# njspix/frender

Hardware: AMD Instinct MI355X
Metric: M reads/sec scanned+classified (96 samples, 8+8bp, n=1) at 1/2/4/8 MI355X (higher is better)
Workload: dtype u8; 1 GPU; BASELINE config 2: 100000000 SYN-v1 reads/GPU, 96 samples, 8+8bp, n=1, R=8 (74 B/record), decoded FASTQ resident in HBM; reads_per_gpu=100000000, bytes_per_record=74, samples=96, nsubs=1, rc=False, unique_codes=1383958, table_checksum=a89b0e2c6adb2921, parallelism=1 GPU

## Files before the change

frender_amd/_lib.py:

```python
from __future__ import annotations

import ctypes as C
import os

import numpy as np

from . import _runtime

torch = None
if _runtime.USE_TORCH:
    try:
        import torch
    except Exception:
        torch = None

HERE = os.path.dirname(os.path.abspath(__file__))
LIB_PATH = os.environ.get("FRENDER_HIP_LIB", os.path.join(HERE, "libfrender_hip.so"))


def source_tree_hash() -> str:
    import hashlib

    h = hashlib.sha256()
    csrc = os.path.join(HERE, "csrc")
# ... 14 lines not shown


class FrenderError(RuntimeError):
    pass


class FileStats(C.Structure):
    _fields_ = [("records", C.c_uint64), ("lines", C.c_uint64), ("new_keys", C.c_uint64),
                ("exotic", C.c_uint64), ("error", C.c_int32), ("utf8_bad", C.c_int32),
                ("error_offset", C.c_uint64)]


class Timing(C.Structure):
    _fields_ = [("scan_launches", C.c_uint64), ("scan_bytes", C.c_uint64), ("scan_ms", C.c_double),
                ("last_scan_ms", C.c_double), ("classify_ms", C.c_double), ("finalize_ms", C.c_double),
                ("log_ms", C.c_double)]


class Tuning(C.Structure):
    _fields_ = [("size", C.c_uint32), ("grid", C.c_int32), ("flush_at", C.c_uint32), ("cold_cap", C.c_uint32),
                ("log", C.c_int32), ("log_min", C.c_uint32), ("log_hot", C.c_uint32), ("chunk_tiles", C.c_uint32),
                ("chunk_tiles_heavy", C.c_uint32), ("ramp", C.c_int32), ("ramp_up_s", C.c_uint32),
                ("ramp_down_s", C.c_uint32), ("ramp_down_pct", C.c_uint32), ("ramp_down_pct_h", C.c_uint32),
                ("spec_commit", C.c_int32), ("nbr", C.c_int32), ("ovf_cap", C.c_uint64)]


if not os.path.exists(LIB_PATH):
    raise ImportError(f"frender_amd: HIP library {LIB_PATH} is not built (run __graft_entry__.build())")
lib = C.CDLL(LIB_PATH)

P = C.c_void_p
u64p = C.POINTER(C.c_uint64)
_SIGS = {
    "fr_create": (P, [C.c_int, C.c_uint64, C.c_uint64]),
    "fr_tuning_defaults": (None, [C.POINTER(Tuning)]),
    "fr_create_tuned": (P, [C.c_int, C.c_uint64, C.c_uint64, C.POINTER(Tuning)]),
    "fr_destroy": (None, [P]),
    "fr_last_error": (C.c_char_p, [P]),
    "fr_get_timing": (C.c_int, [P, C.POINTER(Timing)]),
    "fr_sync": (C.c_int, [P]),
    "fr_set_timing": (C.c_int, [P, C.c_int]),
    "fr_get_diag": (C.c_int, [P, P, C.c_int]),
    "fr_set_sheet": (C.c_int, [P, C.c_int, P, P, P, P, P, P, C.c_int, P, P, P, C.c_int]),
    "fr_reset": (C.c_int, [P]),
    "fr_begin_file": (C.c_int, [P, C.c_int64]),
    "fr_begin_file_at": (C.c_int, [P, C.c_int64, C.c_uint64, C.c_int64]),
    "fr_feed": (C.c_int, [P, P, C.c_uint64]),
# ... 837 lines not shown
```

frender_amd/csrc/fr_api.hip:

```cpp
#include <hip/hip_runtime.h>

#include <algorithm>
#include <cstddef>
#include <cstdio>
#include <cstdlib>
#include <cstring>
#include <string>
#include <thread>
#include <unordered_map>
#include <vector>

#include "../../include/frender_amd.h"
#include "fr_internal.h"

using namespace fr;

static void pinned_copy(u8* dst, const u8* src, u64 n) {
    constexpr u64 PART = 16ull << 20;
    const unsigned hw = std::max(1u, std::thread::hardware_concurrency());
    const u64 k = std::min<u64>({8, hw, n / PART});
    if (k < 2) {
        std::memcpy(dst, src, n);
        return;
    }
    std::vector<std::thread> t;
    const u64 per = (n + k - 1) / k;
    for (u64 i = 1; i < k; ++i) {
        const u64 b = i * per, e = std::min(n, b + per);
        if (b < e) t.emplace_back([=] { std::memcpy(dst + b, src + b, e - b); });
    }
    std::memcpy(dst, src, std::min(n, per));
    for (auto& x : t) x.join();
}

struct fr_ctx {
    int device = 0;
    GSlot* snap = nullptr;
    u64 snap_cap = 0;
    hipStream_t stream = nullptr;
    hipStream_t copy = nullptr;
    std::string err;
    int grid = 0;
    u32 flush_at = NS * 3 / 4;
    u64* cold = nullptr;
    u32 cold_cap = 8192;
    LogEntry* log = nullptr;
    u64 log_cap = 0;
    u32 log_rcap = 0;
    LogEntry* log_sub = nullptr;
    u32 log_scap = 0;
    void* log_temp = nullptr;
    size_t log_temp_bytes = 0;
    u32 log_min = 0;
    u32 log_hot = 0xFFFFFFFFu;
    uint4* rare = nullptr;

    DevState* st = nullptr;
    DevState* h_st = nullptr;
    DevState* h_zero = nullptr;
    u8* h_byte = nullptr;
    u64* h_fin = nullptr;
    HostMirror* h_mir = nullptr;
    HostMirror* d_mir = nullptr;
// ... 168 lines not shown
    while (p < x) p <<= 1;
    return p;
}

static hipError_t fill_async(fr_ctx* ctx, void* dst, int value, size_t bytes) {
    ctx->n_fills++;
    return hipMemsetAsync(dst, value, bytes, ctx->stream);
}

static hipError_t copy_async(fr_ctx* ctx, void* dst, const void* src, size_t bytes, hipMemcpyKind kind) {
    ctx->n_copies++;
    return hipMemcpyAsync(dst, src, bytes, kind, ctx->stream);
}

static int read_state(fr_ctx* ctx) {
    if (ctx->st_fresh && !ctx->st_pending) return FR_OK;
    CK(copy_async(ctx, ctx->h_st, ctx->st, sizeof(DevState), hipMemcpyDeviceToHost));
    CK(hipStreamSynchronize(ctx->stream));
    ctx->st_pending = false;
    ctx->st_fresh = true;
    return FR_OK;
}

static int grow_table(fr_ctx* ctx, bool force_bigger) {
    int rc = read_state(ctx);
    if (rc) return rc;
    const u64 nkeys = ctx->h_st->n_keys;
    const u64 novf = std::min<u64>(ctx->h_st->n_overflow, ctx->tab.ovf_cap);
    if (force_bigger || (nkeys + novf) * 2 > ctx->nslots) {
        u64 ns = ctx->nslots;
        while ((nkeys + novf) * 4 > ns) ns <<= 1;
        if (ns == ctx->nslots) ns <<= 1;
        GSlot* ns_slots = nullptr;
        CK(dalloc(&ns_slots, ns));
        CK(launch_table_init(ns_slots, ns, nullptr, ctx->stream));
        Table t = ctx->tab;
        t.slots = ns_slots;
        t.mask = ns - 1;
        CK(launch_rehash(t, ctx->st, ctx->tab.slots, ctx->nslots, ctx->stream));
        CK(hipStreamSynchronize(ctx->stream));
        CK(hipFree(ctx->tab.slots));
        ctx->tab = t;
        ctx->nslots = ns;
    }
    if (novf) {
        Overflow* old = ctx->tab.ovf;
        Overflow* fresh = nullptr;
        CK(dalloc(&fresh, ctx->tab.ovf_cap));
        ctx->tab.ovf = fresh;
        CK(fill_async(ctx, &ctx->st->n_overflow, 0, sizeof(u64)));
        CK(launch_reinsert_overflow(ctx->tab, ctx->st, old, novf, ctx->stream));
        ctx->st_fresh = false;
        CK(hipStreamSynchronize(ctx->stream));
        CK(hipFree(old));
    }
// ... 318 lines not shown
extern "C" {

void fr_tuning_defaults(fr_tuning* t) {
    if (!t) return;
    const fr_ctx d{};
    std::memset(t, 0, sizeof(*t));
    t->size = sizeof(fr_tuning);
    t->grid = 0;
    t->flush_at = d.flush_at;
    t->cold_cap = d.cold_cap;
    t->log = 1;
    t->log_min = d.log_min;
    t->log_hot = d.log_hot;
    t->chunk_tiles = d.chunk_tiles;
    t->chunk_tiles_heavy = d.chunk_tiles_heavy;
    t->ramp = d.ramp ? 1 : 0;
    t->ramp_up_s = d.ramp_up_s;
    t->ramp_down_s = d.ramp_down_s;
    t->ramp_down_pct = d.ramp_down_pct;
    t->ramp_down_pct_h = d.ramp_down_pct_h;
    t->spec_commit = d.spec_ok ? 1 : 0;
    t->nbr = d.nbr_enabled ? 1 : 0;
    t->ovf_cap = 0;
}

fr_ctx* fr_create(int device, uint64_t chunk_bytes, uint64_t table_slots) {
    return fr_create_tuned(device, chunk_bytes, table_slots, nullptr);
}

fr_ctx* fr_create_tuned(int device, uint64_t chunk_bytes, uint64_t table_slots, const fr_tuning* tuning) {
    fr_tuning t;
    fr_tuning_defaults(&t);
    if (tuning) {
        const size_t n = std::min<size_t>(std::max<uint32_t>(tuning->size, sizeof(uint32_t)), sizeof(fr_tuning));
        std::memcpy((char*)&t + sizeof(uint32_t), (const char*)tuning + sizeof(uint32_t), n - sizeof(uint32_t));
    }
    fr_ctx* ctx = new fr_ctx();
    ctx->device = device;
    auto bad = [&](const char* what, hipError_t e) {
        ctx->err = std::string(what) + ": " + hipGetErrorString(e);
        return ctx;
    };
    hipError_t e;
    if ((e = hipSetDevice(device)) != hipSuccess) return bad("hipSetDevice", e);
    if ((e = hipStreamCreateWithFlags(&ctx->stream, hipStreamNonBlocking)) != hipSuccess) return bad("stream", e);
    if ((e = hipStreamCreateWithFlags(&ctx->copy, hipStreamNonBlocking)) != hipSuccess) return bad("stream", e);
    hipDeviceProp_t prop;
    if ((e = hipGetDeviceProperties(&prop, device)) != hipSuccess) return bad("props", e);
    const int per_cu = chunk_occupancy();
    ctx->grid = t.grid > 0 ? t.grid : prop.multiProcessorCount * per_cu;
    ctx->flush_at = std::min<u32>(t.flush_at, NS);
    ctx->nbr_enabled = t.nbr != 0;
    ctx->cold_cap = std::max<u32>(1024, t.cold_cap);
    ctx->log_min = t.log_min;
    ctx->log_hot = std::max<u32>(1, t.log_hot);
    ctx->chunk_tiles = std::max<u32>(2, t.chunk_tiles);
    ctx->chunk_tiles_heavy = std::max<u32>(2, t.chunk_tiles_heavy);
    ctx->ramp = t.ramp != 0;
    ctx->ramp_up_s = std::max<u32>(1, t.ramp_up_s);
    ctx->ramp_down_s = std::max<u32>(1, t.ramp_down_s);
    ctx->ramp_down_pct = std::min<u32>(100, std::max<u32>(1, t.ramp_down_pct));
    ctx->ramp_down_pct_h = std::min<u32>(100, std::max<u32>(1, t.ramp_down_pct_h));
    ctx->spec_ok = t.spec_commit != 0;
    if ((e = dalloc(&ctx->cold, 2ull * ctx->cold_cap * (u64)ctx->grid)) != hipSuccess) return bad("cold lists", e);
    if ((e = dalloc(&ctx->rare, (u64)RARE_RING * (u64)ctx->grid)) != hipSuccess) return bad("rare rings", e);

    ctx->chunk_bytes = chunk_bytes ? ((chunk_bytes + TILE - 1) / TILE) * TILE : (256ull << 20);
    if (ctx->chunk_bytes > RANGE_MAX) ctx->chunk_bytes = RANGE_MAX;
    ctx->ring_bytes = std::min<u64>(ctx->chunk_bytes, HOST_CHUNK_MAX);
// ... 35 lines not shown
    if ((e = dalloc(&ctx->tab.slots, ctx->nslots)) != hipSuccess) return bad("table", e);
    ctx->tab.mask = ctx->nslots - 1;
    ctx->tab.ovf_cap = t.ovf_cap ? std::max<u64>(t.ovf_cap, 1024) : (1ull << 22);
    ctx->tab.pres_cap = 1ull << 22;
    ctx->tab.exo_cap = 1ull << 20;
    ctx->tab.exo_pool_cap = 64ull << 20;
    if ((e = dalloc(&ctx->tab.ovf, ctx->tab.ovf_cap)) != hipSuccess) return bad("overflow", e);
    if ((e = dalloc(&ctx->tab.pres, ctx->tab.pres_cap)) != hipSuccess) return bad("presence", e);
    if ((e = dalloc(&ctx->tab.exo_ord, ctx->tab.exo_cap)) != hipSuccess) return bad("exotic", e);
    if ((e = dalloc(&ctx->tab.exo_off, ctx->tab.exo_cap)) != hipSuccess) return bad("exotic", e);
    if ((e = dalloc(&ctx->tab.exo_len, ctx->tab.exo_cap)) != hipSuccess) return bad("exotic", e);
    if ((e = dalloc(&ctx->tab.exo_pool, ctx->tab.exo_pool_cap)) != hipSuccess) return bad("exotic", e);
    for (int i = 0; i < 2; ++i) {
        if ((e = hipHostMalloc((void**)&ctx->pin[i], ctx->ring_bytes, hipHostMallocDefault)) != hipSuccess)
            return bad("pinned ring", e);
        if ((e = dalloc(&ctx->dbuf[i], ctx->ring_bytes + 64)) != hipSuccess) return bad("device ring", e);
        if ((e = hipEventCreateWithFlags(&ctx->copied[i], hipEventDisableTiming)) != hipSuccess) return bad("event", e);
        if ((e = hipEventCreateWithFlags(&ctx->consumed[i], hipEventDisableTiming)) != hipSuccess)
            return bad("event", e);
        if ((e = hipEventRecord(ctx->consumed[i], ctx->stream)) != hipSuccess) return bad("event", e);
    }
    if ((e = dalloc(&ctx->d_counter, 1)) != hipSuccess) return bad("counter", e);
    if (fr_reset(ctx) != FR_OK) return ctx;
    ctx->err.clear();
    return ctx;
}

void fr_destroy(fr_ctx* ctx) {
    if (!ctx) return;
    if (ctx->infl) fr_infl_destroy(ctx->infl);
    (void)hipSetDevice(ctx->device);
    if (ctx->stream) (void)hipStreamSynchronize(ctx->stream);
    if (ctx->copy) (void)hipStreamSynchronize(ctx->copy);
    void* dev[] = {ctx->st, ctx->d_tab, ctx->tiles, ctx->tab.slots, ctx->tab.ovf, ctx->tab.pres, ctx->tab.exo_ord,
                   ctx->tab.exo_off, ctx->tab.exo_len, ctx->tab.exo_pool, ctx->dbuf[0], ctx->dbuf[1], ctx->d_sheet,
                   ctx->d_keys, ctx->d_counts, ctx->d_first, ctx->d_keys_s, ctx->d_counts_s,
                   ctx->d_first_s, ctx->d_pos, ctx->d_perm, ctx->d_rank, ctx->d_counter, ctx->d_temp, ctx->d_bins, ctx->d_binbase, ctx->d_arr, ctx->d_rows, ctx->d_pres_u,
                   ctx->d_pres_f, ctx->d_pres_c, ctx->d_m1, ctx->d_m2, ctx->d_row, ctx->d_rm2, ctx->d_rrow, ctx->d_cls, ctx->d_rcls,
                   ctx->d_errw, ctx->d_errf, ctx->d_nbr, ctx->cold, ctx->rare, ctx->chunk_info, ctx->log, ctx->log_sub, ctx->log_temp,
                   ctx->snap};
    for (void* p : dev)
        if (p) (void)hipFree(p);
    if (ctx->h_st) (void)hipHostFree(ctx->h_st);
    if (ctx->h_zero) (void)hipHostFree(ctx->h_zero);
    if (ctx->h_byte) (void)hipHostFree(ctx->h_byte);
    if (ctx->h_fin) (void)hipHostFree(ctx->h_fin);
    if (ctx->h_mir) (void)hipHostFree(ctx->h_mir);
    if (ctx->fin_e0) (void)hipEventDestroy(ctx->fin_e0);
    if (ctx->fin_e1) (void)hipEventDestroy(ctx->fin_e1);
    if (ctx->cls_e0) (void)hipEventDestroy(ctx->cls_e0);
    if (ctx->cls_e1) (void)hipEventDestroy(ctx->cls_e1);
    if (ctx->h_sheet) (void)hipHostFree(ctx->h_sheet);
    if (ctx->h_tab) (void)hipHostFree(ctx->h_tab);
    for (int i = 0; i < 2; ++i) {
        if (ctx->pin[i]) (void)hipHostFree(ctx->pin[i]);
        if (ctx->copied[i]) (void)hipEventDestroy(ctx->copied[i]);
        if (ctx->consumed[i]) (void)hipEventDestroy(ctx->consumed[i]);
    }
    for (auto e : ctx->ev_a) (void)hipEventDestroy(e);
    for (auto e : ctx->ev_b) (void)hipEventDestroy(e);
    for (auto e : ctx->ev_l) (void)hipEventDestroy(e);
    if (ctx->st_ev) (void)hipEventDestroy(ctx->st_ev);
    if (ctx->stream) (void)hipStreamDestroy(ctx->stream);
    if (ctx->copy) (void)hipStreamDestroy(ctx->copy);
    delete ctx;
}

const char* fr_last_error(const fr_ctx* ctx) { return ctx ? ctx->err.c_str() : "null context"; }

int fr_get_diag(fr_ctx* ctx, uint64_t* out, int n) {
    if (int src = settle_finalize(ctx)) return src;
    int rc = read_state(ctx);
    if (rc) return rc;
    const DevState& s = *ctx->h_st;
    const uint64_t v[] = {s.spin_max,   s.spin_total, s.n_keys,   s.n_overflow, s.n_presence, s.n_exotic,
                          (uint64_t)ctx->grid, ctx->nslots, s.stamp[0], s.stamp[1], s.stamp[2], s.stamp[3],
                          s.stamp[4],  s.stamp[5],  s.stamp[6], s.stamp[7], ctx->spec_replays, ctx->exo_replays,
                          s.heavy[ctx->par] ? ctx->chunk_tiles_heavy : ctx->chunk_tiles,
                          s.heavy_launches, ctx->big_rollbacks, ctx->feed_fold_max, ctx->feed_fold_over, ctx->feed_step,
                          ctx->n_fills, ctx->n_copies};
    for (int i = 0; i < n && i < (int)(sizeof(v) / sizeof(v[0])); ++i) out[i] = v[i];
    return FR_OK;
}

int fr_sync(fr_ctx* ctx) {
    CK(hipStreamSynchronize(ctx->stream));
    CK(hipStreamSynchronize(ctx->copy));
    return settle_finalize(ctx);
}

int fr_get_timing(fr_ctx* ctx, fr_timing* out) {
    CK(hipStreamSynchronize(ctx->stream));
    if (int src = settle_finalize(ctx)) return src;
    double tot = 0, last = 0, lg = 0;
    for (size_t i = 0; i < ctx->ev_used; ++i) {
        float ms = 0, ml = 0;
        CK(hipEventElapsedTime(&ms, ctx->ev_a[i], ctx->ev_b[i]));
        CK(hipEventElapsedTime(&ml, ctx->ev_b[i], ctx->ev_l[i]));
        tot += ms;
        last = ms;
        lg += ml;
    }
    out->log_ms = lg;
    out->scan_launches = ctx->scan_launches;
    out->scan_bytes = ctx->scan_bytes;
    out->scan_ms = tot;
    out->last_scan_ms = last;
    out->classify_ms = ctx->classify_ms;
    out->finalize_ms = ctx->finalize_ms;
    return FR_OK;
// ... 67 lines not shown
    ctx->d_name = (int32_t*)(d + o_name);
    ctx->d_cp1 = with_cp ? (u32*)(d + o_cp1) : nullptr;
    ctx->d_cp2 = with_cp ? (u32*)(d + o_cp2) : nullptr;
    ctx->d_cp2rc = with_cp ? (u32*)(d + o_cp2rc) : nullptr;
    ctx->d_cpl1 = with_cp ? (int32_t*)(d + o_l1) : nullptr;
    ctx->d_cpl2 = with_cp ? (int32_t*)(d + o_l2) : nullptr;
    ctx->d_canon = (int32_t*)(d + o_canon);
    ctx->cp_stride = with_cp ? cp_stride : 0;
    ctx->S = S;
    ctx->n_names = n_names;
    auto common = [&](const int32_t* l) {
        if (S == 0) return -1;
        for (int i = 1; i < S; ++i)
            if (l[i] != l[0]) return -2;
        return (int)l[0];
    };
    ctx->L1u = common(idx1_len);
    ctx->L2u = common(idx2_len);
    return FR_OK;
}

int fr_reset(fr_ctx* ctx) {
    if (int src = settle_finalize(ctx)) return src;
    CK(hipSetDevice(ctx->device));
    CK(hipStreamSynchronize(ctx->copy));
    ctx->n_fills = ctx->n_copies = 0;
    if (ctx->st_pending) CK(hipStreamSynchronize(ctx->stream));
    CK(launch_table_init(ctx->tab.slots, ctx->nslots, ctx->st, ctx->stream));
    *ctx->h_st = *ctx->h_zero;
    ctx->st_fresh = true;
    ctx->perfile_clean = true;
    ctx->fold_zero = true;
    ctx->scanning = true;
    ctx->file_open = false;
    ctx->file_tag = 0;
    ctx->first_tag = 0;
    ctx->pres_defer_tag = 0;
    ctx->merged = false;
    ctx->max_file_bytes = 0;
    ctx->par = 0;
    ctx->U = 0;
    ctx->n_pres = 0;
    ctx->n_exo = 0;
    ctx->exo_index.clear();
    ctx->exo_str.clear();
    ctx->exo_codes.clear();
    ctx->exo_pres_code.clear();
    ctx->exo_pres_file.clear();
    ctx->exo_pres_count.clear();
    ctx->last_valid = false;
    ctx->ev_used = 0;
// ... 31 lines not shown
    ctx->file_tag = (u32)file_index + 1u;
    if (!ctx->first_tag) ctx->first_tag = ctx->file_tag;
    ctx->file_offset = byte_base;
    ctx->file_base = byte_base;
    ctx->max_records = max_records > 0 ? max_records : 0;
    ctx->last_byte = -1;
    ctx->carry.clear();
    ctx->sample_done = false;
    ctx->par = 0;
    ctx->file_open = true;
    return FR_OK;
}

static int check_sample(fr_ctx* ctx) {
    if (ctx->max_records <= 0) return FR_OK;
    int rc = read_state(ctx);
    if (rc) return rc;
    const u64 lines = ctx->h_st->lines[ctx->par];
    if (lines + 3 >= 4ull * (u64)ctx->max_records) ctx->sample_done = true;
    return FR_OK;
}

static int ship_slot(fr_ctx* ctx, int slot, u64 n) {
    CK(hipStreamWaitEvent(ctx->copy, ctx->consumed[slot], 0));
    CK(hipMemcpyAsync(ctx->dbuf[slot], ctx->pin[slot], n, hipMemcpyHostToDevice, ctx->copy));
    CK(hipEventRecord(ctx->copied[slot], ctx->copy));
    CK(hipStreamWaitEvent(ctx->stream, ctx->copied[slot], 0));
    int rc = launch_range(ctx, ctx->dbuf[slot], n, n, 1, 0, 0);
    if (rc) return rc;
    CK(hipEventRecord(ctx->consumed[slot], ctx->stream));
    ctx->used[slot] = true;
    return FR_OK;
}

int fr_feed(fr_ctx* ctx, const uint8_t* data, uint64_t len) {
    if (!ctx->file_open) return fail(ctx, FR_ERR_INVALID, "fr_feed: no open file");
    ctx->host_feed = true;
    if (ctx->sample_done) return FR_SAMPLE_DONE;
    if (len) ctx->last_byte = data[len - 1];
    u64 done = 0;
    while (done < len) {
        const int slot = ctx->cur;
        if (ctx->used[slot]) CK(hipEventSynchronize(ctx->copied[slot]));
        u8* pin = ctx->pin[slot];
        const u64 nc = ctx->carry.size();
        if (nc >= ctx->ring_bytes) return fail(ctx, FR_ERR_CAPACITY, "a line is longer than the chunk size");
// ... 50 lines not shown
    const double big_range = (double)std::min<u64>(ctx->chunk_bytes, len);
    const bool fold_room = (u64)ctx->feed_fold_over * 64 <= ctx->feed_fold_max && ctx->feed_step > 0 &&
                           (double)ctx->feed_fold_max * big_range <= 0.85 * AGG_LNS * (double)ctx->feed_step;
    bool big = spec && (!ctx->feed_logged || fold_room) && ctx->feed_keys != ~0ull &&
               (saved.n_keys + ctx->feed_keys) * 2 <= ctx->nslots;
    bool spec_now = spec;
    u64 step = 0, lim_room = ~0ull;
    int last_b = -1;
    for (int attempt = 0; attempt < 12; ++attempt) {
        const bool zero_fold = !ctx->fold_zero;
        bool mirrored = false;
        const u64 lim = std::min<u64>(big ? ctx->chunk_bytes : std::min<u64>(ctx->chunk_bytes, RANGE_FIRST_MAX),
                                      lim_room);
        const u64 nr = (len + lim - 1) / lim;
        step = nr ? (len + nr - 1) / nr : 0;
        ctx->spec_commit = spec_now ? 1u : 0u;
        for (u64 off = 0; off < len; off += step) {
            const u64 n = std::min<u64>(step, len - off);
            rc = launch_range(ctx, dev_data + off, n, len - off, off == 0 ? 1 : 0, 1, off ? 1 : 0, 0,
                              off + n == len, &mirrored, zero_fold && off == 0);
            if (rc) break;
        }
        ctx->spec_commit = 0;
        if (!rc && mirrored) {
            rc = take_mirror(ctx);
            last_b = (int)(ctx->h_mir->last_byte & 0xFFu);
        } else if (!rc) {
            if (len) CK(copy_async(ctx, ctx->h_byte, dev_data + len - 1, 1, hipMemcpyDeviceToHost));
            rc = read_state(ctx);
            if (!rc && len) last_b = *ctx->h_byte;
        }
        if (rc) break;
        const bool spec_bad = spec_now && ctx->h_st->spec_fail;
        const bool room_bad = spec && (ctx->h_st->cap_flags & 2u) && step > RANGE_ROOM_MIN;
        if (!spec_bad && !room_bad) break;
        if (room_bad) {
            big = false;
            lim_room = std::max<u64>(RANGE_ROOM_MIN, ((step / 8) + TILE - 1) / TILE * TILE);
            ctx->grow_sync = true;
            ctx->big_rollbacks++;
        } else {
            spec_now = false;
        }
        if (ctx->nslots != snap_slots) {
            GSlot* fresh = nullptr;
            if ((rc = (dalloc(&fresh, snap_slots) == hipSuccess) ? FR_OK : fail(ctx, FR_ERR_DEVICE, "rollback alloc")))
// ... 79 lines not shown
    if (rc) return fail(ctx, rc, std::string("fr_feed_bgzf: ") + fr_infl_last_error(ctx->infl));
    if (!ok) return FR_OK;
    rc = fr_feed_device(ctx, dev, len);
    if (rc) return rc;
    *decoded = 1;
    if (members) *members = n;
    if (bytes) *bytes = len;
    return FR_OK;
}

int fr_end_file(fr_ctx* ctx, fr_file_stats* out) {
    if (!ctx->file_open) return fail(ctx, FR_ERR_INVALID, "fr_end_file: no open file");
    if (!ctx->carry.empty() && !ctx->sample_done) {
        const int slot = ctx->cur;
        if (ctx->used[slot]) CK(hipEventSynchronize(ctx->copied[slot]));
        std::memcpy(ctx->pin[slot], ctx->carry.data(), ctx->carry.size());
        const u64 n = ctx->carry.size();
        ctx->carry.clear();
        int rc = ship_slot(ctx, slot, n);
        if (rc) return rc;
        ctx->cur ^= 1;
    }
    ctx->carry.clear();
    CK(hipStreamSynchronize(ctx->copy));
    int rc = ctx->host_feed ? settle_exotic(ctx) : FR_OK;
    if (rc) return rc;
    ctx->last_valid = false;
    rc = grow_table(ctx, false);
    if (rc) return rc;
    const bool defer = ctx->file_tag == ctx->first_tag && !ctx->merged && ctx->pres_before == 0 &&
                       ctx->h_st->n_presence == 0;
    if (!defer) {
        rc = ensure_presence_cap(ctx);
        if (rc) return rc;
        ctx->st_fresh = false;
        CK(launch_presence_scan(ctx->tab.slots, ctx->nslots, ctx->file_tag, ctx->tab.pres, ctx->tab.pres_cap,
                                ctx->st, ctx->stream));
    }
    rc = read_state(ctx);
    if (rc) return rc;
    const DevState& s = *ctx->h_st;
    if (s.spin_fail) return fail(ctx, FR_ERR_DEVICE, "tally look-back exceeded its spin bound");
    if (s.cap_flags) return fail(ctx, FR_ERR_CAPACITY, "a device list overflowed (flags " + std::to_string(s.cap_flags) + ")");
    u64 lines = s.lines[ctx->par];
    const bool ended = ctx->last_byte == '\n' || ctx->last_byte == '\r';
    if (ctx->last_byte >= 0 && !ended && !ctx->sample_done) lines += 1;
    u64 records = (lines + 3) / 4;
    if (ctx->max_records > 0 && records > (u64)ctx->max_records) records = (u64)ctx->max_records;
    std::memset(out, 0, sizeof(*out));
    out->records = records;
    out->lines = lines;
    out->new_keys = (defer ? s.n_keys : s.n_presence - ctx->pres_before) + ctx->exo_new_file;
    if (defer) ctx->pres_defer_tag = ctx->file_tag;
    out->exotic = ctx->exo_records_file;
    out->error = FR_SCAN_OK;
    if (s.utf8_bad) {
        out->error = FR_SCAN_UTF8;
        out->utf8_bad = 1;
    }
    if (s.err_nospace != ~0ull) {
        out->error = FR_SCAN_NO_SPACE;
// ... 13 lines not shown
    rc = read_state(ctx);
    if (rc) return rc;
    const u64 nk = ctx->h_st->n_keys;
    if (nk > 0xFFFFFFFFull) return fail(ctx, FR_ERR_CAPACITY, "more than 2^32 unique codes");
    if (nk > ctx->ucap) {
        void* old[] = {ctx->d_keys, ctx->d_counts, ctx->d_first, ctx->d_keys_s, ctx->d_counts_s, ctx->d_first_s,
                       ctx->d_pos, ctx->d_perm, ctx->d_rank, ctx->d_temp};
        for (void* p : old)
            if (p) CK(hipFree(p));
        ctx->d_temp = nullptr;
        ctx->temp_bytes = 0;
        const u64 cap = std::max<u64>(nk + nk / 4, 1024);
        CK(dalloc(&ctx->d_keys, cap));
        CK(dalloc(&ctx->d_counts, cap));
        CK(dalloc(&ctx->d_first, cap));
        CK(dalloc(&ctx->d_keys_s, cap));
        CK(dalloc(&ctx->d_counts_s, cap));
        CK(dalloc(&ctx->d_first_s, cap));
        CK(dalloc(&ctx->d_pos, cap));
        CK(dalloc(&ctx->d_perm, cap));
        CK(dalloc(&ctx->d_rank, cap));
        ctx->ucap = cap;
    }
    if (ctx->timing) CK(hipEventRecord(e0, ctx->stream));
    ctx->fin_timed = ctx->timing;
    BinMap bm{0, 0, 0, 0, 0};
    u64 nbins = 0;
    if (!ctx->merged && ctx->first_tag && ctx->file_tag >= ctx->first_tag) {
        const u64 ntags = (u64)(ctx->file_tag - ctx->first_tag) + 1u;
        bm.span = std::max<u64>(ctx->max_file_bytes, 1);
        bm.first_tag = ctx->first_tag;
        bm.shift = 13;
        const u64 range = ntags * bm.span;
        while (bm.shift < 20 && ((range >> bm.shift) + 1) > (1ull << 21)) ++bm.shift;
        nbins = (range >> bm.shift) + 1;
        if (nbins > (1ull << 21)) nbins = 0;
    }
    if (nbins) {
        bm.nbins = nbins;
        bm.cap = ctx->ucap;
        if (ctx->nslots > ctx->arr_cap) {
            if (ctx->d_arr) CK(hipFree(ctx->d_arr));
            ctx->d_arr = nullptr;
            CK(hipMalloc(&ctx->d_arr, ctx->nslots * sizeof(u32)));
            ctx->arr_cap = ctx->nslots;
        }
// ... 11 lines not shown
            CK(hipMalloc(&ctx->d_bins, cap * sizeof(u32)));
            CK(hipMalloc(&ctx->d_binbase, cap * sizeof(u32)));
            ctx->bins_cap = cap;
            ctx->bins_dirty = true;
        }
        size_t need = 0;
        CK(launch_fin_scan(ctx->d_bins, ctx->d_binbase, nbins + 1, nullptr, &need, ctx->stream));
        if (need > ctx->temp_bytes) {
            if (ctx->d_temp) CK(hipFree(ctx->d_temp));
            CK(hipMalloc(&ctx->d_temp, need));
            ctx->temp_bytes = need;
        }
        size_t tb = ctx->temp_bytes;
        const bool set_uidx = ctx->pres_defer_tag == 0;
        if (ctx->bins_dirty) CK(fill_async(ctx, ctx->d_bins, 0, ctx->bins_cap * sizeof(u32)));
        ctx->bins_dirty = true;
        CK(launch_fin_hist(ctx->tab.slots, ctx->nslots, bm, ctx->d_bins, ctx->d_arr, ctx->stream));
        CK(launch_fin_scan(ctx->d_bins, ctx->d_binbase, nbins + 1, ctx->d_temp, &tb, ctx->stream));
        ctx->h_mir->fin_count = 0;
        CK(launch_fin_scatter(ctx->tab.slots, ctx->nslots, bm, ctx->d_binbase, ctx->d_arr, ctx->d_rows, ctx->d_bins,
                              &ctx->d_mir->fin_count, ctx->stream));
        ctx->bins_dirty = false;
        CK(launch_fin_rank(ctx->tab.slots, nk, bm, ctx->d_binbase, ctx->d_rows, ctx->d_keys_s, ctx->d_counts_s,
                           ctx->d_first_s, set_uidx, ctx->stream));
    } else {
        CK(fill_async(ctx, ctx->d_counter, 0, sizeof(u64)));
        CK(launch_compact(ctx->tab.slots, ctx->nslots, ctx->d_keys, ctx->d_counts, ctx->d_first, ctx->d_pos,
                          ctx->d_counter, ctx->stream));
        int begin_bit = 0, end_bit = 64;
        if (!ctx->merged) {
            begin_bit = 2;
            end_bit = ORD_SHIFT;
            while (end_bit < 64 && ((u64)ctx->file_tag >> (end_bit - ORD_SHIFT)) != 0) ++end_bit;
            if (ctx->file_tag == ctx->first_tag) {
                end_bit = begin_bit + 1;
                while (end_bit < ORD_SHIFT && (ctx->max_file_bytes >> end_bit) != 0) ++end_bit;
            }
        }
        size_t need = 0;
        CK(launch_order(ctx->d_first, ctx->d_pos, nk, ctx->d_first_s, ctx->d_perm, nullptr, &need, begin_bit, end_bit,
                        ctx->stream));
        if (need > ctx->temp_bytes) {
            if (ctx->d_temp) CK(hipFree(ctx->d_temp));
            CK(hipMalloc(&ctx->d_temp, need));
            ctx->temp_bytes = need;
        }
        size_t tb = ctx->temp_bytes;
        if (nk)
            CK(launch_order(ctx->d_first, ctx->d_pos, nk, ctx->d_first_s, ctx->d_perm, ctx->d_temp, &tb, begin_bit,
                            end_bit, ctx->stream));
        CK(launch_gather(ctx->d_perm, nk, ctx->d_keys, ctx->d_counts, ctx->d_keys_s, ctx->d_counts_s, ctx->d_rank,
                         ctx->stream));
        CK(launch_set_uidx(ctx->tab.slots, ctx->tab.mask, ctx->d_keys_s, nk, ctx->d_rank, ctx->stream));
    }
    const u64 np = ctx->pres_defer_tag ? nk : std::min<u64>(ctx->h_st->n_presence, ctx->tab.pres_cap);
    if (np > ctx->pmap_cap) {
        if (ctx->d_pres_u) CK(hipFree(ctx->d_pres_u));
        if (ctx->d_pres_f) CK(hipFree(ctx->d_pres_f));
        if (ctx->d_pres_c) CK(hipFree(ctx->d_pres_c));
        CK(dalloc(&ctx->d_pres_u, np));
        CK(dalloc(&ctx->d_pres_f, np));
        CK(dalloc(&ctx->d_pres_c, np));
        ctx->pmap_cap = np;
    }
    if (ctx->pres_defer_tag)
        CK(launch_presence_one_file(ctx->d_counts_s, np, ctx->pres_defer_tag, ctx->d_pres_u, ctx->d_pres_f,
                                    ctx->d_pres_c, ctx->stream));
    else
        CK(launch_presence_map(ctx->tab.slots, ctx->tab.mask, ctx->tab.pres, np, ctx->d_pres_u, ctx->d_pres_f,
                               ctx->d_pres_c, ctx->stream));
    ctx->fin_binned = nbins != 0;
    *ctx->h_fin = 0;
    if (!nbins) CK(copy_async(ctx, ctx->h_fin, ctx->d_counter, sizeof(u64), hipMemcpyDeviceToHost));
    CK(hipEventRecord(e1, ctx->stream));
    ctx->fin_pending = true;
    ctx->fin_expect = nk;
    ctx->U = nk;
    ctx->n_pres = np;
    ctx->n_exo = ctx->exo_codes.size();
    if (n_unique) *n_unique = ctx->U;
    if (n_presence) *n_presence = ctx->n_pres;
    if (n_exotic) *n_exotic = ctx->n_exo;
    return FR_OK;
}

int fr_get_unique(fr_ctx* ctx, uint64_t* keys, uint64_t* counts, uint64_t* first_ordinal) {
    if (int src = settle_finalize(ctx)) return src;
    const u64 n = ctx->U;
    if (!n) return FR_OK;
    if (keys) CK(hipMemcpy(keys, ctx->d_keys_s, n * 8, hipMemcpyDeviceToHost));
    if (counts) CK(hipMemcpy(counts, ctx->d_counts_s, n * 8, hipMemcpyDeviceToHost));
    if (first_ordinal) CK(hipMemcpy(first_ordinal, ctx->d_first_s, n * 8, hipMemcpyDeviceToHost));
    return FR_OK;
// ... 343 lines not shown
```

frender_amd/csrc/fr_internal.h:

```cpp
#pragma once
#include <hip/hip_runtime.h>
#include <stdint.h>

#include <vector>

namespace fr {

typedef uint8_t u8;
typedef uint16_t u16;
typedef uint32_t u32;
typedef uint64_t u64;
typedef int64_t i64;

constexpr int WG = 256;
constexpr int SEG = 64;
constexpr int TILE = 64 * SEG;
constexpr int TSTEP = TILE - SEG;
#ifndef FR_LOG_NS
#define FR_LOG_NS 10
#endif
constexpr int LOG_NS = FR_LOG_NS;
constexpr int NS = 1 << LOG_NS;
#ifndef FR_LPROBE
#define FR_LPROBE 2
// ... 240 lines not shown
                        void* temp, size_t* temp_bytes, int begin_bit, int end_bit, hipStream_t s);
hipError_t launch_gather(const u32* perm, u64 n, const u64* keys, const u64* counts, u64* keys_o,
                         u64* counts_o, u32* rank, hipStream_t s);
hipError_t launch_presence_one_file(const u64* counts, u64 n, u32 tag, u32* uidx, u32* file_idx, u64* snap,
                                    hipStream_t s);
hipError_t launch_presence_map(const GSlot* slots, u64 mask, const Presence* pres, u64 n, u32* uidx,
                               u32* file_idx, u64* snap, hipStream_t s);
struct BinMap {
    u64 span;
    u32 first_tag;
    u32 shift;
    u64 nbins;
    u64 cap;
};
struct alignas(32) FinRow {
    u64 first, key, count;
    u32 slot, pad;
};
hipError_t launch_fin_hist(const GSlot* slots, u64 nslots, const BinMap& m, u32* cnt, u32* arr, hipStream_t s);
hipError_t launch_fin_scan(const u32* cnt, u32* base, u64 n, void* temp, size_t* temp_bytes, hipStream_t s);
hipError_t launch_fin_scatter(const GSlot* slots, u64 nslots, const BinMap& m, const u32* base, const u32* arr,
                              FinRow* rows, u32* cnt, u64* fin_out, hipStream_t s);
hipError_t launch_fin_rank(GSlot* slots, u64 nk, const BinMap& m, const u32* base, const FinRow* rows, u64* keys_o,
                           u64* counts_o, u64* first_o, bool set_uidx, hipStream_t s);
hipError_t launch_classify(const u64* keys, const u64* counts, u64 n, SheetArgs sh, int nsubs, int rc,
                           ClassOut o, const NbrMap& nm, u64* zero_next, u32 zero_n, u64* err_flag, hipStream_t s);
u64 nbr_codes_per_row(int L, int nsubs);
hipError_t launch_nbr_build(const SheetArgs& sh, const int32_t* canon, int nsubs, int rc, const NbrMap& nm,
                            hipStream_t s);
hipError_t launch_classify_cp(int n, const u32* q1, const int32_t* q1len, const u32* q2, const int32_t* q2len,
                              int stride, int S, const u32* s1, const int32_t* s1len, const u32* s2,
                              const int32_t* s2len, const u32* s2rc, const int32_t* name, int nsubs, int rc,
                              ClassOut o, hipStream_t s);
hipError_t launch_presence_scan(const GSlot* slots, u64 n, u32 tag, Presence* pres, u64 cap, DevState* st,
                                hipStream_t s);
hipError_t launch_merge(Table t, DevState* st, const u64* keys, const u64* counts, const u64* first, u64 n,
                        hipStream_t s);
hipError_t launch_partition_rows(const u64* keys, const u64* counts_in, const u64* first, u64 n, u32 world,
                                 u64* counts, u64* cursor, u64* rows, hipStream_t s);
hipError_t launch_merge_rows(Table t, DevState* st, const u64* rows, u64 n, hipStream_t s);
hipError_t launch_log_aggregate(Table t, DevState* st, const LogEntry* log, u32 rcap, LogEntry* sub, u32 scap,
                                u32 file_tag, u64 file_offset, HostMirror* mir, const u8* last_byte, hipStream_t s);
size_t log_aggregate_temp_bytes();
hipError_t launch_synth(u8* out, u64 r0, u64 n, int R, u64 seed, const u8* idx1, const u8* idx2, int S, int L1,
                        int L2, hipStream_t s);

struct BgzfMember {
// ... 9 lines not shown
```

frender_amd/csrc/fr_kernels.hip:

```cpp
#include <algorithm>
#include <cstdlib>
#include <cstring>

#include <rocprim/rocprim.hpp>

#include "fr_internal.h"

namespace fr {

#if defined(FR_STAMPS) && FR_STAMPS == 1
#define FR_STAMP_DECL u64 st_[8] = {0, 0, 0, 0, 0, 0, 0, 0}; u64 tq_ = __builtin_amdgcn_s_memtime();
#define FR_STAMP(i) do { const u64 n_ = __builtin_amdgcn_s_memtime(); st_[i] += n_ - tq_; tq_ = n_; } while (0)
#define FR_STAMP_FLUSH(k0) do { st_[6] = __builtin_amdgcn_s_memtime() - (k0); \
    if ((threadIdx.x & 63) == 0) for (int i_ = 0; i_ < 8; ++i_) atomicAdd((unsigned long long*)&a.st->stamp[i_], \
        (unsigned long long)st_[i_]); } while (0)
#else
#define FR_STAMP_DECL
#define FR_STAMP(i) do { } while (0)
#define FR_STAMP_FLUSH(k0) do { } while (0)
#endif

#if defined(FR_STAMPS) && FR_STAMPS == 2
#define FR_CSTAMP(i) do { const u64 n_ = __builtin_amdgcn_s_memtime(); cst_[i] += n_ - cq_; cq_ = n_; } while (0)
#else
// ... 2277 lines not shown
    const u64 i = blockIdx.x * (u64)blockDim.x + threadIdx.x;
    for (u64 j = i; j <= m.nbins; j += (u64)gridDim.x * blockDim.x) cnt[j] = 0;
    if (i == 0 && fin_out) {
        *fin_out = base[m.nbins];
        __threadfence_system();
    }
    if (i >= n) return;
    const u32 k = arr[i];
    if (k == 0xFFFFFFFFu) return;
    const uint4 w0 = *(const uint4*)&slots[i];
    const uint4 w1 = *((const uint4*)&slots[i] + 1);
    const u64 first = ((u64)w1.y << 32) | w1.x;
    const u32 q = base[ord_bin(m, first)] + k;
    if (q < m.cap) {
        typedef u32 u32x4 __attribute__((ext_vector_type(4)));
        u32x4* d = (u32x4*)&rows[q];
        d[0] = u32x4{w1.x, w1.y, w0.x, w0.y};
        d[1] = u32x4{w0.z, w0.w, (u32)i, 0u};
    }
}

__global__ __launch_bounds__(256) void fin_rank_kernel(GSlot* slots, u64 nk, BinMap m, const u32* base,
                                                       const FinRow* rows, u64* keys_o, u64* counts_o, u64* first_o,
                                                       int set_uidx) {
    const u64 q = blockIdx.x * (u64)blockDim.x + threadIdx.x;
    if (q >= nk) return;
    const FinRow row = rows[q];
    const u64 b = ord_bin(m, row.first);
    const u32 lo = base[b], hi = (u32)min((u64)base[b + 1], m.cap);
    u32 r = 0;
    for (u32 j = lo; j < hi; ++j) {
        const u64 fj = rows[j].first;
        r += (fj < row.first || (fj == row.first && rows[j].slot < row.slot)) ? 1u : 0u;
    }
    const u32 out = lo + r;
    if (out >= nk) return;
    keys_o[out] = row.key;
    counts_o[out] = row.count;
    first_o[out] = row.first;
    if (set_uidx) slots[row.slot].uidx = out;
}

static unsigned lane_grid(u64 n) { return (unsigned)std::max<u64>(1, (n + 255) / 256); }

hipError_t launch_fin_hist(const GSlot* slots, u64 nslots, const BinMap& m, u32* cnt, u32* arr, hipStream_t s) {
    hipLaunchKernelGGL(fin_hist_kernel, dim3(lane_grid(nslots)), dim3(256), 0, s, slots, nslots, m, cnt, arr);
    return hipGetLastError();
}

hipError_t launch_fin_scan(const u32* cnt, u32* base, u64 n, void* temp, size_t* temp_bytes, hipStream_t s) {
    return rocprim::exclusive_scan(temp, *temp_bytes, cnt, base, 0u, (size_t)n, rocprim::plus<u32>(), s);
}

hipError_t launch_fin_scatter(const GSlot* slots, u64 nslots, const BinMap& m, const u32* base, const u32* arr,
                              FinRow* rows, u32* cnt, u64* fin_out, hipStream_t s) {
    hipLaunchKernelGGL(fin_scatter_kernel, dim3(lane_grid(nslots)), dim3(256), 0, s, slots, nslots, m, base, arr, rows,
                       cnt, fin_out);
    return hipGetLastError();
}

hipError_t launch_fin_rank(GSlot* slots, u64 nk, const BinMap& m, const u32* base, const FinRow* rows, u64* keys_o,
                           u64* counts_o, u64* first_o, bool set_uidx, hipStream_t s) {
    if (!nk) return hipSuccess;
    hipLaunchKernelGGL(fin_rank_kernel, dim3(lane_grid(nk)), dim3(256), 0, s, slots, nk, m, base, rows, keys_o,
                       counts_o, first_o, set_uidx ? 1 : 0);
    return hipGetLastError();
}

__global__ void merge_kernel(Table t, DevState* st, const u64* keys, const u64* counts, const u64* first, u64 n) {
    u32 made = 0;
    for (u64 i = blockIdx.x * (u64)blockDim.x + threadIdx.x; i < n; i += (u64)gridDim.x * blockDim.x)
        made += global_insert(t, st, keys[i], counts[i], first[i], 0u) ? 1u : 0u;
    add_created(st, made);
}

constexpr int PART_MAX = 1024;
__device__ __forceinline__ u32 owner_rank(u64 key, u32 world) {
    return (u32)(((key * 0x9E3779B97F4A7C15ull) >> 40) & 0xFFFFFFull) % world;
}
__global__ __launch_bounds__(256) void part_count_kernel(const u64* keys, u64 n, u32 world, u64* counts) {
    __shared__ u32 h[PART_MAX];
    for (u32 i = threadIdx.x; i < world; i += 256) h[i] = 0;
    __syncthreads();
    for (u64 i = blockIdx.x * 256ull + threadIdx.x; i < n; i += (u64)gridDim.x * 256ull) atomicAdd(&h[owner_rank(keys[i], world)], 1u);
    __syncthreads();
    for (u32 i = threadIdx.x; i < world; i += 256)
        if (h[i]) atomicAdd((unsigned long long*)&counts[i], (unsigned long long)h[i]);
}
// ... 690 lines not shown
```

include/frender_amd.h:

```cpp
#ifndef FRENDER_AMD_H
#define FRENDER_AMD_H

#include <stddef.h>
#include <stdint.h>

#ifdef __cplusplus
extern "C" {
#endif

#define FR_OK 0
#define FR_ERR_INVALID 1
#define FR_ERR_HIP 2
#define FR_ERR_CAPACITY 3
#define FR_ERR_DEVICE 4
#define FR_ERR_IO 6

#define FR_SCAN_OK 0
#define FR_SCAN_NO_SPACE 1
#define FR_SCAN_UTF8 2

#define FR_UNDETERMINED 0
#define FR_INDEX_HOP 1
#define FR_DEMUXABLE 2
#define FR_AMBIGUOUS 3
// ... 19 lines not shown
    double finalize_ms;
    double log_ms;
} fr_timing;

fr_ctx* fr_create(int device, uint64_t chunk_bytes, uint64_t table_slots);
typedef struct fr_tuning {
    uint32_t size;
    int32_t grid;
    uint32_t flush_at;
    uint32_t cold_cap;
    int32_t log;
    uint32_t log_min;
    uint32_t log_hot;
    uint32_t chunk_tiles;
    uint32_t chunk_tiles_heavy;
    int32_t ramp;
    uint32_t ramp_up_s;
    uint32_t ramp_down_s;
    uint32_t ramp_down_pct;
    uint32_t ramp_down_pct_h;
    int32_t spec_commit;
    int32_t nbr;
    uint64_t ovf_cap;
} fr_tuning;
void fr_tuning_defaults(fr_tuning* t);
fr_ctx* fr_create_tuned(int device, uint64_t chunk_bytes, uint64_t table_slots, const fr_tuning* t);
void fr_destroy(fr_ctx* ctx);
const char* fr_last_error(const fr_ctx* ctx);
int fr_get_timing(fr_ctx* ctx, fr_timing* out);
int fr_set_timing(fr_ctx* ctx, int on);
int fr_sync(fr_ctx* ctx);
int fr_get_diag(fr_ctx* ctx, uint64_t* out, int n);

int fr_set_sheet(fr_ctx* ctx, int S,
                 const uint64_t* idx1_packed, const int32_t* idx1_len,
                 const uint64_t* idx2_packed, const int32_t* idx2_len,
                 const uint64_t* idx2rc_packed, const int32_t* name_id, int n_names,
                 const uint32_t* idx1_cp, const uint32_t* idx2_cp, const uint32_t* idx2rc_cp,
                 int cp_stride);

int fr_reset(fr_ctx* ctx);
int fr_begin_file(fr_ctx* ctx, int64_t max_records );
int fr_begin_file_at(fr_ctx* ctx, int64_t file_index, uint64_t byte_base, int64_t max_records);
#define FR_SAMPLE_DONE 5
int fr_feed(fr_ctx* ctx, const uint8_t* data, uint64_t len);
typedef struct fr_gz fr_gz;
// ... 127 lines not shown
```

Measured before the change: 40630 M reads/s.

## Double-buffer hash table with background clear on low-priority stream; fuse presence map into rank

Keeps a spare hash-table allocation that is re-initialised on a separate low-priority stream while other work runs, so a reset swaps tables instead of clearing the full table inline. It also folds the per-file presence map writes into the fin_rank kernel when finalize is binned, which removes a separate launch, and it skips redundant copy-stream syncs and hipSetDevice calls on reset. The cost is a second table's worth of device memory, extra event and stream bookkeeping, and possible contention from the background clear with the main kernels.

After: 40840 M reads/s, median of 2. No clear change (+0.5%).

```diff
diff --git a/frender_amd/_lib.py b/frender_amd/_lib.py
--- a/frender_amd/_lib.py
+++ b/frender_amd/_lib.py
@@ -60,7 +60,8 @@
                 ("log", C.c_int32), ("log_min", C.c_uint32), ("log_hot", C.c_uint32), ("chunk_tiles", C.c_uint32),
                 ("chunk_tiles_heavy", C.c_uint32), ("ramp", C.c_int32), ("ramp_up_s", C.c_uint32),
                 ("ramp_down_s", C.c_uint32), ("ramp_down_pct", C.c_uint32), ("ramp_down_pct_h", C.c_uint32),
-                ("spec_commit", C.c_int32), ("nbr", C.c_int32), ("ovf_cap", C.c_uint64)]
+                ("spec_commit", C.c_int32), ("nbr", C.c_int32), ("ovf_cap", C.c_uint64),
+                ("spare_table", C.c_int32)]
 
 
 if not os.path.exists(LIB_PATH):
diff --git a/frender_amd/csrc/fr_api.hip b/frender_amd/csrc/fr_api.hip
--- a/frender_amd/csrc/fr_api.hip
+++ b/frender_amd/csrc/fr_api.hip
@@ -39,6 +39,17 @@
     u64 snap_cap = 0;
     hipStream_t stream = nullptr;
     hipStream_t copy = nullptr;
+    bool copy_touched = false;
+    hipStream_t clear = nullptr;
+    GSlot* spare = nullptr;
+    u64 spare_slots = 0;
+    enum { SPARE_NONE, SPARE_DIRTY, SPARE_QUEUED };
+    int spare_state = SPARE_NONE;
+    hipEvent_t spare_ev = nullptr;
+    hipEvent_t gate_ev = nullptr;
+    bool spare_on = true;
+    bool spare_failed = false;
+    u64 resets = 0;
     std::string err;
     int grid = 0;
     u32 flush_at = NS * 3 / 4;
@@ -253,6 +264,27 @@
     return FR_OK;
 }
 
+static int queue_spare_clear(fr_ctx* ctx) {
+    if (ctx->spare_state != fr_ctx::SPARE_DIRTY) return FR_OK;
+    CK(hipEventRecord(ctx->gate_ev, ctx->stream));
+    CK(hipStreamWaitEvent(ctx->clear, ctx->gate_ev, 0));
+    CK(launch_table_init(ctx->spare, ctx->spare_slots, nullptr, ctx->clear));
+    CK(hipEventRecord(ctx->spare_ev, ctx->clear));
+    ctx->spare_state = fr_ctx::SPARE_QUEUED;
+    return FR_OK;
+}
+
+static int drop_spare(fr_ctx* ctx) {
+    if (!ctx->spare) return FR_OK;
+    CK(hipStreamSynchronize(ctx->clear));
+    GSlot* old = ctx->spare;
+    ctx->spare = nullptr;
+    ctx->spare_slots = 0;
+    ctx->spare_state = fr_ctx::SPARE_NONE;
+    CK(hipFree(old));
+    return FR_OK;
+}
+
 static int grow_table(fr_ctx* ctx, bool force_bigger) {
     int rc = read_state(ctx);
     if (rc) return rc;
@@ -262,6 +294,7 @@
         u64 ns = ctx->nslots;
         while ((nkeys + novf) * 4 > ns) ns <<= 1;
         if (ns == ctx->nslots) ns <<= 1;
+        if ((rc = drop_spare(ctx))) return rc;
         GSlot* ns_slots = nullptr;
         CK(dalloc(&ns_slots, ns));
         CK(launch_table_init(ns_slots, ns, nullptr, ctx->stream));
@@ -626,6 +659,7 @@
     t->spec_commit = d.spec_ok ? 1 : 0;
     t->nbr = d.nbr_enabled ? 1 : 0;
     t->ovf_cap = 0;
+    t->spare_table = d.spare_on ? 1 : 0;
 }
 
 fr_ctx* fr_create(int device, uint64_t chunk_bytes, uint64_t table_slots) {
@@ -649,6 +683,13 @@
     if ((e = hipSetDevice(device)) != hipSuccess) return bad("hipSetDevice", e);
     if ((e = hipStreamCreateWithFlags(&ctx->stream, hipStreamNonBlocking)) != hipSuccess) return bad("stream", e);
     if ((e = hipStreamCreateWithFlags(&ctx->copy, hipStreamNonBlocking)) != hipSuccess) return bad("stream", e);
+    int prio_least = 0, prio_greatest = 0;
+    if ((e = hipDeviceGetStreamPriorityRange(&prio_least, &prio_greatest)) != hipSuccess) return bad("stream", e);
+    if ((e = hipStreamCreateWithPriority(&ctx->clear, hipStreamNonBlocking, prio_least)) != hipSuccess)
+        return bad("stream", e);
+    if ((e = hipEventCreateWithFlags(&ctx->spare_ev, hipEventDisableTiming)) != hipSuccess) return bad("event", e);
+    if ((e = hipEventCreateWithFlags(&ctx->gate_ev, hipEventDisableTiming)) != hipSuccess) return bad("event", e);
+    ctx->spare_on = t.spare_table != 0;
     hipDeviceProp_t prop;
     if ((e = hipGetDeviceProperties(&prop, device)) != hipSuccess) return bad("props", e);
     const int per_cu = chunk_occupancy();
@@ -730,6 +771,7 @@
     }
     if ((e = dalloc(&ctx->d_counter, 1)) != hipSuccess) return bad("counter", e);
     if (fr_reset(ctx) != FR_OK) return ctx;
+    ctx->resets = 0;
     ctx->err.clear();
     return ctx;
 }
@@ -740,7 +782,8 @@
     (void)hipSetDevice(ctx->device);
     if (ctx->stream) (void)hipStreamSynchronize(ctx->stream);
     if (ctx->copy) (void)hipStreamSynchronize(ctx->copy);
-    void* dev[] = {ctx->st, ctx->d_tab, ctx->tiles, ctx->tab.slots, ctx->tab.ovf, ctx->tab.pres, ctx->tab.exo_ord,
+    if (ctx->clear) (void)hipStreamSynchronize(ctx->clear);
+    void* dev[] = {ctx->spare, ctx->st, ctx->d_tab, ctx->tiles, ctx->tab.slots, ctx->tab.ovf, ctx->tab.pres, ctx->tab.exo_ord,
                    ctx->tab.exo_off, ctx->tab.exo_len, ctx->tab.exo_pool, ctx->dbuf[0], ctx->dbuf[1], ctx->d_sheet,
                    ctx->d_keys, ctx->d_counts, ctx->d_first, ctx->d_keys_s, ctx->d_counts_s,
                    ctx->d_first_s, ctx->d_pos, ctx->d_perm, ctx->d_rank, ctx->d_counter, ctx->d_temp, ctx->d_bins, ctx->d_binbase, ctx->d_arr, ctx->d_rows, ctx->d_pres_u,
@@ -769,6 +812,9 @@
     for (auto e : ctx->ev_b) (void)hipEventDestroy(e);
     for (auto e : ctx->ev_l) (void)hipEventDestroy(e);
     if (ctx->st_ev) (void)hipEventDestroy(ctx->st_ev);
+    if (ctx->spare_ev) (void)hipEventDestroy(ctx->spare_ev);
+    if (ctx->gate_ev) (void)hipEventDestroy(ctx->gate_ev);
+    if (ctx->clear) (void)hipStreamDestroy(ctx->clear);
     if (ctx->stream) (void)hipStreamDestroy(ctx->stream);
     if (ctx->copy) (void)hipStreamDestroy(ctx->copy);
     delete ctx;
@@ -794,6 +840,8 @@
 int fr_sync(fr_ctx* ctx) {
     CK(hipStreamSynchronize(ctx->stream));
     CK(hipStreamSynchronize(ctx->copy));
+    ctx->copy_touched = false;
+    CK(hipStreamSynchronize(ctx->clear));
     return settle_finalize(ctx);
 }
 
@@ -907,11 +955,40 @@
 
 int fr_reset(fr_ctx* ctx) {
     if (int src = settle_finalize(ctx)) return src;
-    CK(hipSetDevice(ctx->device));
-    CK(hipStreamSynchronize(ctx->copy));
+    int dev_now = -1;
+    if (hipGetDevice(&dev_now) != hipSuccess || dev_now != ctx->device) CK(hipSetDevice(ctx->device));
+    if (ctx->copy_touched) {
+        CK(hipStreamSynchronize(ctx->copy));
+        ctx->copy_touched = false;
+    }
     ctx->n_fills = ctx->n_copies = 0;
     if (ctx->st_pending) CK(hipStreamSynchronize(ctx->stream));
-    CK(launch_table_init(ctx->tab.slots, ctx->nslots, ctx->st, ctx->stream));
+    if (ctx->spare_on && !ctx->spare_failed && ctx->resets >= 1) {
+        if (ctx->spare && ctx->spare_slots != ctx->nslots) {
+            if (int src = drop_spare(ctx)) return src;
+        }
+        if (!ctx->spare) {
+            if (dalloc(&ctx->spare, ctx->nslots) != hipSuccess) {
+                (void)hipGetLastError();
+                ctx->spare = nullptr;
+                ctx->spare_failed = true;
+            } else {
+                ctx->spare_slots = ctx->nslots;
+                ctx->spare_state = fr_ctx::SPARE_DIRTY;
+            }
+        }
+    }
+    ctx->resets++;
+    if (ctx->spare) {
+        CK(launch_table_init(ctx->tab.slots, 0, ctx->st, ctx->stream));
+        if (int src = queue_spare_clear(ctx)) return src;
+        CK(hipStreamWaitEvent(ctx->stream, ctx->spare_ev, 0));
+        std::swap(ctx->tab.slots, ctx->spare);
+        ctx->h_tab->slots = ctx->tab.slots;
+        ctx->spare_state = fr_ctx::SPARE_DIRTY;
+    } else {
+        CK(launch_table_init(ctx->tab.slots, ctx->nslots, ctx->st, ctx->stream));
+    }
     *ctx->h_st = *ctx->h_zero;
     ctx->st_fresh = true;
     ctx->perfile_clean = true;
@@ -989,6 +1066,7 @@
 }
 
 static int ship_slot(fr_ctx* ctx, int slot, u64 n) {
+    ctx->copy_touched = true;
     CK(hipStreamWaitEvent(ctx->copy, ctx->consumed[slot], 0));
     CK(hipMemcpyAsync(ctx->dbuf[slot], ctx->pin[slot], n, hipMemcpyHostToDevice, ctx->copy));
     CK(hipEventRecord(ctx->copied[slot], ctx->copy));
@@ -1085,6 +1163,7 @@
             if (rc) break;
         }
         ctx->spec_commit = 0;
+        if (!rc) rc = queue_spare_clear(ctx);
         if (!rc && mirrored) {
             rc = take_mirror(ctx);
             last_b = (int)(ctx->h_mir->last_byte & 0xFFu);
@@ -1210,7 +1289,10 @@
         ctx->cur ^= 1;
     }
     ctx->carry.clear();
-    CK(hipStreamSynchronize(ctx->copy));
+    if (ctx->copy_touched) {
+        CK(hipStreamSynchronize(ctx->copy));
+        ctx->copy_touched = false;
+    }
     int rc = ctx->host_feed ? settle_exotic(ctx) : FR_OK;
     if (rc) return rc;
     ctx->last_valid = false;
@@ -1225,6 +1307,7 @@
         CK(launch_presence_scan(ctx->tab.slots, ctx->nslots, ctx->file_tag, ctx->tab.pres, ctx->tab.pres_cap,
                                 ctx->st, ctx->stream));
     }
+    if ((rc = queue_spare_clear(ctx))) return rc;
     rc = read_state(ctx);
     if (rc) return rc;
     const DevState& s = *ctx->h_st;
@@ -1284,6 +1367,19 @@
         CK(dalloc(&ctx->d_rank, cap));
         ctx->ucap = cap;
     }
+    const u64 np = ctx->pres_defer_tag ? nk : std::min<u64>(ctx->h_st->n_presence, ctx->tab.pres_cap);
+    if (np > ctx->pmap_cap) {
+        if (ctx->d_pres_u) CK(hipFree(ctx->d_pres_u));
+        if (ctx->d_pres_f) CK(hipFree(ctx->d_pres_f));
+        if (ctx->d_pres_c) CK(hipFree(ctx->d_pres_c));
+        ctx->d_pres_u = ctx->d_pres_f = nullptr;
+        ctx->d_pres_c = nullptr;
+        ctx->pmap_cap = 0;
+        CK(dalloc(&ctx->d_pres_u, np));
+        CK(dalloc(&ctx->d_pres_f, np));
+        CK(dalloc(&ctx->d_pres_c, np));
+        ctx->pmap_cap = np;
+    }
     if (ctx->timing) CK(hipEventRecord(e0, ctx->stream));
     ctx->fin_timed = ctx->timing;
     BinMap bm{0, 0, 0, 0, 0};
@@ -1341,7 +1437,8 @@
                               &ctx->d_mir->fin_count, ctx->stream));
         ctx->bins_dirty = false;
         CK(launch_fin_rank(ctx->tab.slots, nk, bm, ctx->d_binbase, ctx->d_rows, ctx->d_keys_s, ctx->d_counts_s,
-                           ctx->d_first_s, set_uidx, ctx->stream));
+                           ctx->d_first_s, set_uidx, ctx->pres_defer_tag, ctx->d_pres_u, ctx->d_pres_f, ctx->d_pres_c,
+                           ctx->stream));
     } else {
         CK(fill_async(ctx, ctx->d_counter, 0, sizeof(u64)));
         CK(launch_compact(ctx->tab.slots, ctx->nslots, ctx->d_keys, ctx->d_counts, ctx->d_first, ctx->d_pos,
@@ -1372,22 +1469,15 @@
                          ctx->stream));
         CK(launch_set_uidx(ctx->tab.slots, ctx->tab.mask, ctx->d_keys_s, nk, ctx->d_rank, ctx->stream));
     }
-    const u64 np = ctx->pres_defer_tag ? nk : std::min<u64>(ctx->h_st->n_presence, ctx->tab.pres_cap);
-    if (np > ctx->pmap_cap) {
-        if (ctx->d_pres_u) CK(hipFree(ctx->d_pres_u));
-        if (ctx->d_pres_f) CK(hipFree(ctx->d_pres_f));
-        if (ctx->d_pres_c) CK(hipFree(ctx->d_pres_c));
-        CK(dalloc(&ctx->d_pres_u, np));
-        CK(dalloc(&ctx->d_pres_f, np));
-        CK(dalloc(&ctx->d_pres_c, np));
-        ctx->pmap_cap = np;
-    }
-    if (ctx->pres_defer_tag)
-        CK(launch_presence_one_file(ctx->d_counts_s, np, ctx->pres_defer_tag, ctx->d_pres_u, ctx->d_pres_f,
-                                    ctx->d_pres_c, ctx->stream));
-    else
+    if (ctx->pres_defer_tag) {
+        if (!nbins)
+            CK(launch_presence_one_file(ctx->d_counts_s, np, ctx->pres_defer_tag, ctx->d_pres_u, ctx->d_pres_f,
+                                        ctx->d_pres_c, ctx->stream));
+    } else {
         CK(launch_presence_map(ctx->tab.slots, ctx->tab.mask, ctx->tab.pres, np, ctx->d_pres_u, ctx->d_pres_f,
                                ctx->d_pres_c, ctx->stream));
+    }
+    if ((rc = queue_spare_clear(ctx))) return rc;
     ctx->fin_binned = nbins != 0;
     *ctx->h_fin = 0;
     if (!nbins) CK(copy_async(ctx, ctx->h_fin, ctx->d_counter, sizeof(u64), hipMemcpyDeviceToHost));
diff --git a/frender_amd/csrc/fr_internal.h b/frender_amd/csrc/fr_internal.h
--- a/frender_amd/csrc/fr_internal.h
+++ b/frender_amd/csrc/fr_internal.h
@@ -286,7 +286,8 @@
 hipError_t launch_fin_scatter(const GSlot* slots, u64 nslots, const BinMap& m, const u32* base, const u32* arr,
                               FinRow* rows, u32* cnt, u64* fin_out, hipStream_t s);
 hipError_t launch_fin_rank(GSlot* slots, u64 nk, const BinMap& m, const u32* base, const FinRow* rows, u64* keys_o,
-                           u64* counts_o, u64* first_o, bool set_uidx, hipStream_t s);
+                           u64* counts_o, u64* first_o, bool set_uidx, u32 pres_tag, u32* pres_u, u32* pres_f,
+                           u64* pres_c, hipStream_t s);
 hipError_t launch_classify(const u64* keys, const u64* counts, u64 n, SheetArgs sh, int nsubs, int rc,
                            ClassOut o, const NbrMap& nm, u64* zero_next, u32 zero_n, u64* err_flag, hipStream_t s);
 u64 nbr_codes_per_row(int L, int nsubs);
diff --git a/frender_amd/csrc/fr_kernels.hip b/frender_amd/csrc/fr_kernels.hip
--- a/frender_amd/csrc/fr_kernels.hip
+++ b/frender_amd/csrc/fr_kernels.hip
@@ -2323,7 +2323,8 @@
 
 __global__ __launch_bounds__(256) void fin_rank_kernel(GSlot* slots, u64 nk, BinMap m, const u32* base,
                                                        const FinRow* rows, u64* keys_o, u64* counts_o, u64* first_o,
-                                                       int set_uidx) {
+                                                       int set_uidx, u32 pres_tag, u32* pres_u, u32* pres_f,
+                                                       u64* pres_c) {
     const u64 q = blockIdx.x * (u64)blockDim.x + threadIdx.x;
     if (q >= nk) return;
     const FinRow row = rows[q];
@@ -2339,6 +2340,11 @@
     keys_o[out] = row.key;
     counts_o[out] = row.count;
     first_o[out] = row.first;
+    if (pres_tag) {
+        pres_u[out] = out;
+        pres_f[out] = pres_tag - 1u;
+        pres_c[out] = row.count & ((1ull << (64 - PRES_TAG_BITS)) - 1ull);
+    }
     if (set_uidx) slots[row.slot].uidx = out;
 }
 
@@ -2361,10 +2367,11 @@
 }
 
 hipError_t launch_fin_rank(GSlot* slots, u64 nk, const BinMap& m, const u32* base, const FinRow* rows, u64* keys_o,
-                           u64* counts_o, u64* first_o, bool set_uidx, hipStream_t s) {
+                           u64* counts_o, u64* first_o, bool set_uidx, u32 pres_tag, u32* pres_u, u32* pres_f,
+                           u64* pres_c, hipStream_t s) {
     if (!nk) return hipSuccess;
     hipLaunchKernelGGL(fin_rank_kernel, dim3(lane_grid(nk)), dim3(256), 0, s, slots, nk, m, base, rows, keys_o,
-                       counts_o, first_o, set_uidx ? 1 : 0);
+                       counts_o, first_o, set_uidx ? 1 : 0, pres_tag, pres_u, pres_f, pres_c);
     return hipGetLastError();
 }
 
diff --git a/include/frender_amd.h b/include/frender_amd.h
--- a/include/frender_amd.h
+++ b/include/frender_amd.h
@@ -65,6 +65,7 @@
     int32_t spec_commit;
     int32_t nbr;
     uint64_t ovf_cap;
+    int32_t spare_table;
 } fr_tuning;
 void fr_tuning_defaults(fr_tuning* t);
 fr_ctx* fr_create_tuned(int device, uint64_t chunk_bytes, uint64_t table_slots, const fr_tuning* t);
```
